# ahmetumutdurmus/zaremba

Hardware: NVIDIA H100
Metric: tokens/sec (and valid perplexity) Large-LSTM 1500h at 1/2/4/8 H100 vs ref CPU (higher is better)
Workload: dtype f16 operands, f32 accumulate/state

## Files before the change

### zaremba_b200/csrc/adam_tc.cu

```cuda
#include "update_tile.cuh"

namespace zrb {

__device__ __forceinline__ void adam_elem(float& p, float& g, float& m, float& v, float coef, const AdamScalars& k) {
    g = __fmul_rn(g, coef);
    m = __fadd_rn(__fmul_rn(k.beta1, m), __fmul_rn(k.omb1, g));
    v = __fadd_rn(__fmul_rn(k.beta2, v), __fmul_rn(k.omb2, __fmul_rn(g, g)));
    const float denom = __fadd_rn(__fdiv_rn(__fsqrt_rn(v), k.bc2s), k.eps);
    p = __fsub_rn(p, __fmul_rn(k.step_size, __fdiv_rn(m, denom)));
}

struct AdamRule : NoTileRule {
    float* m;
    float* v;
    AdamScalars k;
    const float* scalars;
    float coef;
    static constexpr bool kMayWriteG = true;
    static constexpr int kWhhMinBlocks = 3;
    template <int VEC> struct Tile { float m[kTileRows][VEC], v[kTileRows][VEC]; };
    __device__ __forceinline__ void init() { coef = scalars[1]; }
    template <int VEC>
    __device__ __forceinline__ void apply(int64_t, float (&)[VEC], float (&)[VEC]) const {}
    template <int VEC> __device__ __forceinline__ void load(int64_t off, int e, Tile<VEC>& t) const {
        load_vec<VEC>(m + off, t.m[e]);
        load_vec<VEC>(v + off, t.v[e]);
    }
    template <int VEC>
    __device__ __forceinline__ void finish(int e, float (&pv)[VEC], float (&gv)[VEC], Tile<VEC>& t) const {
#pragma unroll
        for (int x = 0; x < VEC; ++x) adam_elem(pv[x], gv[x], t.m[e][x], t.v[e][x], coef, k);
    }
    template <int VEC> __device__ __forceinline__ void store(int64_t off, int e, const Tile<VEC>& t) const {
        store_vec<VEC>(m + off, t.m[e]);
        store_vec<VEC>(v + off, t.v[e]);
    }
};

int update_pack_adam(float* p, float* g, float* m, float* v, const AdamScalars& k, int rows, int cols,
                     const float* scalars, const WeightImages& img, bool write_g, cudaStream_t s, bool pdl) {
    AdamRule rule;
    rule.m = m; rule.v = v; rule.k = k; rule.scalars = scalars; rule.coef = 0.f;
    return update_pack_rule(p, g, rows, cols, rule, (uintptr_t)m | (uintptr_t)v, img, write_g, s, pdl);
}

constexpr int kAdamListThreads = 256;
constexpr int kAdamListBlocks = 148 * 16;

struct AdamRuns {
    float* p[kMaxTensors];
    float* g[kMaxTensors];
    float* m[kMaxTensors];
    float* v[kMaxTensors];
    int64_t n[kMaxTensors];
};

template <bool WRITE_G>
__global__ void __launch_bounds__(kAdamListThreads) adam_list_kernel(AdamRuns d, AdamScalars k,
                                                                     const float* __restrict__ scalars) {
    float* __restrict__ p = d.p[blockIdx.y];
    float* __restrict__ g = d.g[blockIdx.y];
    float* __restrict__ m = d.m[blockIdx.y];
    float* __restrict__ v = d.v[blockIdx.y];
    const int64_t n = d.n[blockIdx.y];
    const float coef = scalars[1];
    const int64_t tid = (int64_t)blockIdx.x * blockDim.x + threadIdx.x, stride = (int64_t)gridDim.x * blockDim.x;
    int64_t j0 = 0;
    if (((((uintptr_t)p) | ((uintptr_t)g) | ((uintptr_t)m) | ((uintptr_t)v)) & 15) == 0) {
        const int64_t n4 = n >> 2;
        for (int64_t i = tid; i < n4; i += stride) {
            float pv[4], gv[4], mv[4], vv[4];
            load_vec<4>(g + 4 * i, gv);
            load_vec<4>(p + 4 * i, pv);
            load_vec<4>(m + 4 * i, mv);
            load_vec<4>(v + 4 * i, vv);
#pragma unroll
// ... 41 lines not shown
```

### zaremba_b200/csrc/average_tc.cu

```cuda
#include "update_tile.cuh"

namespace zrb {

__device__ __forceinline__ float avg_elem(float a, float p, float mu, int first) {
    return first ? p : __fadd_rn(a, __fmul_rn(__fsub_rn(p, a), mu));
}

struct AvgRule : SgdRule {
    float* a;
    float mu;
    int first;
    static constexpr int kWhhMinBlocks = 3;
    template <int VEC> struct Tile { float v[kTileRows][VEC]; };
    template <int VEC> __device__ __forceinline__ void load(int64_t off, int e, Tile<VEC>& t) const {
        load_vec<VEC>(a + off, t.v[e]);
    }
    template <int VEC>
    __device__ __forceinline__ void finish(int e, float (&pv)[VEC], float (&)[VEC], Tile<VEC>& t) const {
#pragma unroll
        for (int x = 0; x < VEC; ++x) t.v[e][x] = avg_elem(t.v[e][x], pv[x], mu, first);
    }
    template <int VEC> __device__ __forceinline__ void store(int64_t off, int e, const Tile<VEC>& t) const {
        store_vec<VEC>(a + off, t.v[e]);
    }
};

struct SwapRule : NoTileRule {
    static constexpr bool kMayWriteG = true;
    static constexpr int kWhhMinBlocks = 4;
    __device__ __forceinline__ void init() {}
    template <int VEC>
    __device__ __forceinline__ void apply(int64_t, float (&pv)[VEC], float (&gv)[VEC]) const {
#pragma unroll
        for (int x = 0; x < VEC; ++x) { const float t = pv[x]; pv[x] = gv[x]; gv[x] = t; }
    }
};

int update_pack_avg(float* p, float* g, float* a, float mu, bool first, int rows, int cols, float lr,
                    const float* scalars, const WeightImages& img, bool write_g, cudaStream_t s, bool pdl) {
    AvgRule rule;
    rule.lr = lr; rule.scalars = scalars; rule.coef = 0.f;
    rule.a = a; rule.mu = mu; rule.first = first ? 1 : 0;
    return update_pack_rule(p, g, rows, cols, rule, (uintptr_t)a, img, write_g, s, pdl);
}

int swap_pack(float* p, float* a, int rows, int cols, const WeightImages& img, cudaStream_t s) {
    return update_pack_rule(p, a, rows, cols, SwapRule{}, 0, img, true, s, false);
}

constexpr int kListThreads = 256;
constexpr int kListBlocks = 148 * 16;

struct AvgRuns {
    float* p[kMaxTensors];
    float* g[kMaxTensors];
    float* a[kMaxTensors];
    int64_t n[kMaxTensors];
};

static int avg_runs(const TensorList& tl, float* const* a, AvgRuns* d, int* bx) {
    int k = 0;
    int64_t longest = 0;
    for (int t = 0; t < tl.count; ++t) {
        if (tl.n[t] == 0) continue;
        d->p[k] = tl.p[t]; d->g[k] = tl.g[t]; d->a[k] = a[t]; d->n[k] = tl.n[t];
        longest = tl.n[t] > longest ? tl.n[t] : longest;
        ++k;
    }
    int64_t b = (longest / 4 + kListThreads - 1) / kListThreads;
    if (b < 1) b = 1;
    const int cap = kListBlocks / (k > 0 ? k : 1);
    *bx = (int)(b > cap ? cap : b);
    return k;
}

template <bool SGD, bool WRITE_G>
// ... 99 lines not shown
```

### zaremba_b200/csrc/engine_tc.cu

```cuda
#include "engine.h"
#include <stdlib.h>
#include <string.h>

#include "tc_kernels.h"

struct GridBarrier {
    unsigned int* word = nullptr;
    unsigned int base = 0;
    template <typename Launch>
    int claim(int T, int nCTA, cudaStream_t s, Launch&& launch) {
        const unsigned int arrivals = (unsigned int)T * (unsigned int)nCTA;
        if (base > 0xF0000000u - arrivals) {
            ZRB_CUDA(cudaMemsetAsync(word, 0, sizeof(unsigned int), s));
            base = 0;
        }
        ZRB_TRY(launch(word, base));
        base += arrivals;
        return ZRB_OK;
    }
};

struct zrb_tc_state {
    int Xp[ZRB_MAX_LAYERS + 1] = {}, G4p[ZRB_MAX_LAYERS] = {}, Vp = 0;
    int Fp = 0;
// ... 292 lines not shown
    }
    ms.m[ms.n++] = {1 + 4 * L, V, K ? c->width[0] : c->width[L], L, WeightMatrix::kFcW};
    return ms;
}
static WeightImages tc_images(zrb_ctx* c, const WeightMatrix& m, const zrb_tc_state::WhhImage& whh) {
    zrb_tc_state* t = c->tc;
    switch (m.kind) {
        case WeightMatrix::kWhh: return t->w_hh_images(m.item, whh);
        case WeightMatrix::kWih: return t->w_ih_images(m.item);
        case WeightMatrix::kFcW: return t->fc_w_images();
        case WeightMatrix::kPrior: return t->row_image(t->head_w_h + (size_t)t->Ua * t->Xp[m.item], t->Xp[m.item]);
        default: return t->row_image(t->head_w_h, t->Xp[m.item]);
    }
}
static TensorList tc_without_matrices(const zrb_ctx* c, const TensorList& tl) {
    TensorList rest = tl;
    for (const WeightMatrix& m : tc_matrices(c)) rest.n[m.i] = 0;
    return rest;
}
static bool tc_streams_aligned(const TensorList& tl, float* const* x1 = nullptr, float* const* x2 = nullptr) {
    uintptr_t all = 0;
    for (int i = 0; i < tl.count; ++i)
        all |= (uintptr_t)tl.p[i] | (uintptr_t)tl.g[i] | (x1 ? (uintptr_t)x1[i] : 0) | (x2 ? (uintptr_t)x2[i] : 0);
    return (all & 3) == 0;
}
static void tc_images_current(zrb_ctx* c, const zrb_params* p) {
    zrb_tc_state* t = c->tc;
    t->wg_ok = false;
    c->weights_version++;
    note_packed(c, p);
}

static int tc_update_matrix(zrb_ctx* c, const WeightMatrix& m, const TensorList& tl, float lr, const AvgStep* avg,
                            const AdamStep* adam, bool pdl, cudaStream_t s) {
    zrb_tc_state::WhhImage whh;
    if (c->p_wd > 0.f) whh.kind = zrb_tc_state::kWhhStale;
    const WeightImages img = tc_images(c, m, whh);
    float *p = tl.p[m.i], *g = tl.g[m.i];
    if (adam)
        return update_pack_adam(p, g, adam->m[m.i], adam->v[m.i], adam->k, m.rows, m.cols, c->scalars, img,
                                c->keep_clipped, s, pdl);
    if (!avg) return update_pack(p, g, m.rows, m.cols, lr, c->scalars, img, c->keep_clipped, s, pdl);
    return update_pack_avg(p, g, avg->a[m.i], avg->mu, avg->first, m.rows, m.cols, lr, c->scalars, img, c->keep_clipped,
                           s, pdl);
}

static int tc_issue_update(zrb_ctx* c, int item, bool pdl, cudaStream_t s) {
    zrb_tc_state* t = c->tc;
    if (!(t->upd_pending & (1u << item))) return ZRB_OK;
    t->upd_pending &= ~(1u << item);
    const AvgStep* avg = t->upd_avg_on ? &t->upd_avg : nullptr;
    const AdamStep* adam = t->upd_adam_on ? &t->upd_adam : nullptr;
    for (const WeightMatrix& m : tc_matrices(c))
        if (m.item == item) ZRB_TRY(tc_update_matrix(c, m, t->upd_tl, t->upd_lr, avg, adam, pdl, s));
    return ZRB_OK;
}

int tc_flush_updates(zrb_ctx* c, cudaStream_t s) {
    zrb_tc_state* t = c->tc;
    if (!t || !t->upd_pending) return ZRB_OK;
    ProfScope ps(c, ZRB_PROF_CLIP_SGD, s);
    for (int item = 1; item <= c->cfg.layers; ++item) ZRB_TRY(tc_issue_update(c, item, false, s));
    return ZRB_OK;
}

static int tc_mos_head(zrb_ctx* c, const zrb_params* p, int rows, float* logp, cudaStream_t s) {
    zrb_tc_state* t = c->tc;
    const int L = c->cfg.layers, V = c->cfg.vocab, K = c->experts, E = c->width[0], H = c->width[L];
    const int N = c->T * c->B, Xl = t->Xp[L], Ep = pad64(E);
    ProfScope ps(c, ZRB_PROF_PROJ_FWD, s);
    Gemm head;
    head.A = {t->x_h[L] + (size_t)(N - rows) * Xl, Xl}; head.B = {t->head_w_h, Xl};
    head.C = t->ua; head.ldc = t->HW; head.M = rows; head.N = t->Ua + K; head.K = H;
    ZRB_TRY(gemm_f16_tc(head, s));
    ZRB_TRY(mos_latent_fwd(t->ua, t->HW, mos_of(p)->latent_b, t->lat_h, Ep, rows, K, E, N - rows, mos_mask(c), s));
    Gemm logits;
    logits.A = {t->lat_h, Ep}; logits.B = {t->fc_w_h, t->Fp};
    logits.C = t->logits; logits.ldc = V; logits.M = rows * K; logits.N = V; logits.K = E; logits.bias = p->fc_b;
    ZRB_TRY(gemm_f16_tc(logits, s));
    ZRB_TRY(mos_lse(t->logits, rows * K, V, t->lse, s));
    if (logp) ZRB_TRY(mos_logp(t->logits, t->lse, t->ua, t->HW, t->Ua, rows, K, V, logp, V, s));
    return ZRB_OK;
}

int tc_forward(zrb_ctx* c, const zrb_params* p, const int64_t* x, const zrb_states* in, const zrb_states* out,
               float* scores, cudaStream_t s, bool last_only) {
    zrb_tc_state* t = c->tc;
    const int L = c->cfg.layers, V = c->cfg.vocab, T = c->T, B = c->B, N = T * B;
    const bool ride = t->upd_pending && t->in_train_step && t->fplan[0].ok && pdl_beside_rec(c);
    if (t->upd_pending && !ride) ZRB_TRY(tc_flush_updates(c, s));
    ZRB_TRY(tc_pack_weights(c, p, s));
    {
        FwdPrep fp = {};
        for (int l = 0; l < L; ++l) {
            fp.in_h[l] = in->h[l]; fp.in_c[l] = in->c[l]; fp.h0s[l] = c->h0s[l]; fp.c0s[l] = c->c0s[l];
// ... 12 lines not shown
        ZRB_TRY(embed_dropout_fwd(p->embed_w, x, nullptr, t->x_h[0], t->Xp[0], N, c->width[0], V, site_mask(c, 0), ed_mask(c), s,
                                  through ? t->upd_tl.g[tc_matrices(c).fc_w().i] : nullptr, t->upd_lr, c->scalars));
    }
    for (int l = 0; l < L; ++l) {
        const int In = c->width[l], H = c->width[l + 1], Xi = t->Xp[l], Hp = t->Xp[l + 1];
        const size_t bh = (size_t)B * H * sizeof(float);
        const RecPlan& fplan = t->fplan[l];
        float* G = c->gates[l];
        if (!whh_current(c, l)) {
            ProfScope ps(c, ZRB_PROF_PACK, s);
            ZRB_TRY(tc_pack_whh(c, p->w_hh[l], l, false, s));
        }
        {
            ProfScope ps(c, ZRB_PROF_GEMM_IN, s);
            Gemm xw;
            xw.A = {t->x_h[l], Xi}; xw.B = {t->w_ih_h[l], Xi};
            xw.C = G; xw.ldc = 4 * H; xw.M = N; xw.N = 4 * H; xw.K = In; xw.bias = p->b_ih[l]; xw.bias2 = p->b_hh[l];
            ZRB_TRY(gemm_f16_tc(xw, s));
        }
        MaskSrc m = site_mask(c, l + 1), rm = rec_mask(c, l);
        const ZoneoutSrc zo = zoneout_src(c, l);
        const bool reg_h = t->in_train_step && reg_on(c) && l == L - 1;
        ProfScope ps(c, ZRB_PROF_REC_FWD, s);
        if (fplan.ok) {
            ZRB_TRY(t->fwd_bar.claim(T, fplan.nCTA, s, [&](unsigned int* word, unsigned int base) {
                RecFwdArgs a = {};
                a.w_img = t->w_img_f[l]; a.h0_img = t->h0_img[l]; a.h_img = t->h_img; a.gates = G; a.c0 = c->c0s[l];
                a.cst = c->cst[l]; a.h_last = out->h[l]; a.c_last = out->c[l]; a.hprev_h = t->hprev_h[l];
                a.y_h = t->x_h[l + 1]; a.h_f32 = reg_h ? c->hraw[l] : nullptr; a.counter = word; a.base = base;
                a.T = T; a.B = B; a.H = H; a.Hp = Hp; a.m = m; a.rm = rm; a.trace = t->trace;
                a.zo = zo; a.h0 = c->h0s[l]; a.ctil = c->ctil[l];
                return lstm_rec_fwd(fplan, tc_watchdog(c), a, s);
            }));
            if (ride) ZRB_TRY(tc_issue_update(c, l + 1, true, s));
            continue;
        }
        for (int tt = 0; tt < T; ++tt) {
            const float* c_prev = tt ? c->cst[l] + (size_t)(tt - 1) * B * H : c->c0s[l];
            float* Gt = G + (size_t)tt * B * 4 * H;
            Gemm hw;
            hw.A = {t->hprev_h[l] + (size_t)tt * B * Hp, Hp}; hw.B = {t->w_hh_h[l], Hp};
            hw.C = Gt; hw.ldc = 4 * H; hw.M = B; hw.N = 4 * H; hw.K = H; hw.accumulate = true;
            ZRB_TRY(gemm_f16_tc(hw, s));
            const float* h_prev = tt ? c->hraw[l] + (size_t)(tt - 1) * B * H : c->h0s[l];
            ZRB_TRY(lstm_cell_fwd_tc(Gt, c_prev, c->cst[l] + (size_t)tt * B * H, c->hraw[l] + (size_t)tt * B * H,
                                     t->hprev_h[l] + (size_t)(tt + 1) * B * Hp, t->x_h[l + 1] + (size_t)tt * B * Hp, Hp, B,
                                     H, (int64_t)tt * B * H, (int64_t)N * H, m, rm, s, zo.on ? &zo : nullptr, h_prev,
                                     zo.on ? c->ctil[l] + (size_t)tt * B * H : nullptr));
        }
        ZRB_CUDA(cudaMemcpyAsync(out->h[l], c->hraw[l] + (size_t)(T - 1) * B * H, bh, cudaMemcpyDeviceToDevice, s));
        ZRB_CUDA(cudaMemcpyAsync(out->c[l], c->cst[l] + (size_t)(T - 1) * B * H, bh, cudaMemcpyDeviceToDevice, s));
    }
    if (scores && c->experts) return tc_mos_head(c, p, last_only ? B : N, t->head_loss_only ? nullptr : scores, s);
    if (scores) {
        ProfScope ps(c, ZRB_PROF_PROJ_FWD, s);
        const int rows = last_only ? B : N;
        const int Xl = t->Xp[L];
        Gemm proj;
        proj.A = {t->x_h[L] + (size_t)(N - rows) * Xl, Xl}; proj.B = {t->fc_w_h, Xl};
        proj.C = scores; proj.ldc = V; proj.M = rows; proj.N = V; proj.K = c->width[L]; proj.bias = p->fc_b;
        ZRB_TRY(gemm_f16_tc(proj, s));
    }
    return ZRB_OK;
}

const __half* tc_last_layer_image(const zrb_ctx* c) { return c->tc->x_h[c->cfg.layers]; }

// ... 418 lines not shown
    TensorList rest = tc_without_matrices(c, tl);
    if (rows_only && !adam) rest.n[0] = 0;
    TensorList dense = gemm_norm ? rest : tl;
    if (rows_only) dense.n[0] = 0;
    if (c->tied && gemm_norm) {
        ZRB_TRY(grad_norm(dense, max_norm, c->partials, c->scalars, norm_out, s, true, t->wg_slots));
    } else if (rows_only) {
        ZRB_TRY(embed_first_table(c->emb_prev_ids, c->emb_first, c->emb_prev_n, V, s));
        ZRB_TRY(embed_rows_sumsq(tl.g[0], c->emb_prev_ids, c->emb_first, c->emb_prev_n, E, V,
                                 c->partials + norm_partials_base(), kNormExtra, s));
        ZRB_TRY(grad_norm(dense, max_norm, c->partials, c->scalars, norm_out, s, true, gemm_norm ? t->wg_slots : 0));
        if (!adam)
            ZRB_TRY(embed_rows_update(tl.p[0], tl.g[0], c->emb_prev_ids, c->emb_first, c->emb_prev_n, E, V, lr,
                                      c->scalars, c->keep_clipped, s));
        if (avg) {
            TensorList e{};
            e.p[0] = tl.p[0]; e.n[0] = tl.n[0]; e.count = 1;
            ZRB_TRY(avg_apply(e, avg->a, avg->mu, avg->first, s));
        }
    } else {
        ZRB_TRY(grad_norm(tl, max_norm, c->partials, c->scalars, norm_out, s));
    }
    const bool lazy = c->lazy_update && t->persistent() && pdl_beside_rec(c);
    if (lazy) {
        t->upd_tl = tl;
        t->upd_lr = lr;
        t->upd_avg_on = avg != nullptr;
        if (avg) t->upd_avg = *avg;
        t->upd_adam_on = adam != nullptr;
        if (adam) t->upd_adam = *adam;
    }
    for (const WeightMatrix& m : tc_matrices(c)) {
        if (lazy && m.item >= 1 && !(adam && c->tied && m.item == L)) t->upd_pending |= 1u << m.item;
        else ZRB_TRY(tc_update_matrix(c, m, tl, lr, avg, adam, false, s));
    }
    if (adam) ZRB_TRY(adam_apply(rest, *adam, c->scalars, c->keep_clipped, s));
    else if (avg) ZRB_TRY(sgd_avg_apply(rest, avg->a, lr, c->scalars, c->keep_clipped, avg->mu, avg->first, s));
    else ZRB_TRY(sgd_apply(rest, lr, c->scalars, c->keep_clipped, s));
    tc_images_current(c, p);
    return ZRB_OK;
}

int tc_dyneval_update(zrb_ctx* c, const zrb_params* p, const TensorList& tl, float* const* tg, float* const* r,
                      const DynArgs& a, cudaStream_t s) {
    ZRB_TRY(tc_flush_updates(c, s));
    ProfScope ps(c, ZRB_PROF_CLIP_SGD, s);
    if (!tc_streams_aligned(tl, tg, r)) {
        ZRB_TRY(dyneval_apply(tl, tg, r, a, s));
        c->weights_version++;
        return ZRB_OK;
    }
    for (const WeightMatrix& m : tc_matrices(c))
        ZRB_TRY(update_pack_dyn(tl.p[m.i], tl.g[m.i], tg[m.i], r ? r[m.i] : nullptr, m.rows, m.cols, a,
                                tc_images(c, m, {}), s));
    ZRB_TRY(dyneval_apply(tc_without_matrices(c, tl), tg, r, a, s));
    tc_images_current(c, p);
    return ZRB_OK;
}

int tc_swap_average(zrb_ctx* c, const zrb_params* p, const TensorList& tl, float* const* a, cudaStream_t s) {
    ZRB_TRY(tc_flush_updates(c, s));
    ProfScope ps(c, ZRB_PROF_PACK, s);
    if (!tc_streams_aligned(tl, a)) {
        ZRB_TRY(swap_apply(tl, a, s));
        c->weights_version++;
        return ZRB_OK;
    }
// ... 8 lines not shown
```

### zaremba_b200/csrc/lstm_rec_bwd.cu

```cuda
#include <stdlib.h>

#include "lstm_rec_bwd.cuh"

namespace zrb {

__global__ void pack_whh_bwd_kernel(const float* __restrict__ W, __half* __restrict__ img, int H, int UC, int G, int KcS,
                                    int S, int nCluster, MaskSrc m) {
    __shared__ __half tile[8][8 * 128];
    const int warp_in_block = threadIdx.x >> 5, lane = threadIdx.x & 31;
    const int CS = 4 * S;
    const long long total = (long long)nCluster * CS * KcS;
    for (long long w = (long long)blockIdx.x * 8 + warp_in_block; w < total; w += (long long)gridDim.x * 8) {
        const int kcl = (int)(w % KcS);
        const int r = (int)((w / KcS) % CS);
        const int cl = (int)(w / ((long long)KcS * CS));
        const int gate = r / S, khalf = r % S;
        __half* t = tile[warp_in_block];
        const int rows8 = G * 8;
        if (m.active) {
            for (int idx = lane * 4; idx < 8 * rows8; idx += 128) {
                const int e = idx / rows8, u0 = idx % rows8;
                const int k = (khalf * KcS + kcl) * 8 + e, j0 = cl * UC + u0;
                const size_t row = (size_t)gate * H + k;
                float mul[4] = {0.f, 0.f, 0.f, 0.f};
                if (k < H && u0 < UC && j0 < H) mask_mul4_at(m, row * H + j0, mul);
#pragma unroll
                for (int q = 0; q < 4; ++q) {
                    const int u = u0 + q, j = j0 + q;
                    t[u * 8 + e] = __float2half_rn((k < H && u < UC && j < H) ? W[row * H + j] * mul[q] : 0.f);
                }
            }
        } else {
            for (int idx = lane; idx < 8 * rows8; idx += 32) {
                int e = idx / rows8, u = idx % rows8;
                int k = (khalf * KcS + kcl) * 8 + e, j = cl * UC + u;
                float v = (k < H && u < UC && j < H) ? W[((size_t)gate * H + k) * H + j] : 0.f;
                t[u * 8 + e] = __float2half_rn(v);
            }
        }
        __syncwarp();
        __half* dst = img + (((size_t)cl * CS + r) * KcS + kcl) * ((size_t)G * 64);
        for (int idx = lane; idx < rows8 * 8; idx += 32) dst[idx] = t[idx];
        __syncwarp();
    }
}

int rec_bwd_plan(int H, int B, RecPlan* plan) {
    int nsm = tc_num_sms();
    plan->GB = (B + 7) / 8;
    plan->ok = 0;
    plan->KS = 1;
    if (plan->GB * 8 > 32) return ZRB_OK;
    if (H >= 256) {
        const int Kp = (H + 31) / 32 * 32, Kc = Kp / 8, KcS = Kc / 2, GBi = (plan->GB + 1) / 2 * 2;
        for (int pass = 0; pass < 2; ++pass)
            for (int U = 16; U >= 1; --U) {
                const int UC = 8 * U;
                if (UC > 128) continue;
                const int ncl = (H + UC - 1) / UC;
                if (ncl * 8 > nsm) break;
                if (U * B > (pass == 0 ? 1 : kRecMaxCell) * kRecEpiThreads) continue;
                const int G = UC / 8;
                const size_t smem = rec_smem_bytes(KcS, G, GBi);
                if (smem <= 227 * 1024 && 8 * U * (GBi * 8 + 4) <= 2 * 64 * (GBi * 8 + 1)) {
                    if (rec_max_clusters((const void*)lstm_rec_bwd_kernel<2, false>, 8, (int)smem, 8 * 64) < ncl) continue;
                    plan->KS = 2; plan->U = U; plan->G = G; plan->nCTA = ncl * 8; plan->smem = (int)smem;
                    plan->Kc = Kc; plan->KcS = KcS; plan->GBi = GBi;
                    return rec_plan_finish(plan, (const void*)lstm_rec_bwd_kernel<2, false>, 8);
                }
            }
    }
    int Kp = (H + 15) / 16 * 16;
    plan->Kc = Kp / 8;
    plan->KcS = plan->Kc;
    plan->GBi = plan->GB;
    int max_clusters = (nsm - 16) / 4;
    for (int U = 16; U >= 1; --U) {
        int UC = 4 * U;
        if (UC % 8) continue;
        int ncl = (H + UC - 1) / UC;
        if (ncl > max_clusters) break;
        int G = UC / 8;
        size_t smem = rec_smem_bytes(plan->Kc, G, plan->GB);
        if (smem <= 227 * 1024 && U * B <= kRecMaxCell * kRecEpiThreads) {
            plan->U = U; plan->G = G; plan->nCTA = ncl * 4; plan->smem = (int)smem;
            return rec_plan_finish(plan, (const void*)lstm_rec_bwd_kernel<1, false>, 4);
        }
    }
    return ZRB_OK;
}

int pack_whh_bwd(const float* W, __half* img, int H, const RecPlan& p, cudaStream_t s, MaskSrc m) {
    const int CS = 4 * p.KS;
    pack_whh_bwd_kernel<<<tc_num_sms() * 4, 256, 0, s>>>(W, img, H, CS * p.U, p.G, p.KcS, p.KS, p.nCTA / CS, m);
// ... 23 lines not shown
```

### zaremba_b200/csrc/lstm_rec_fwd.cu

```cuda
#include <stdlib.h>

#include "lstm_rec_fwd.cuh"

namespace zrb {

__global__ void pack_whh_fwd_kernel(const float* __restrict__ W, __half* __restrict__ img, int H, int UC, int G, int KcS,
                                    int KS, int nCTA, MaskSrc m) {
    const size_t per_cta = (size_t)KcS * G * 64;
    const size_t total = per_cta * nCTA;
    if (m.active) {
        for (size_t idx = ((size_t)blockIdx.x * blockDim.x + threadIdx.x) * 4; idx < total;
             idx += (size_t)gridDim.x * blockDim.x * 4) {
            int cta = (int)(idx / per_cta);
            size_t r0 = idx % per_cta;
            int e0 = (int)(r0 & 7), r = (int)((r0 >> 3) & 7);
            int g = (int)((r0 >> 6) % G), kcl = (int)((r0 >> 6) / G);
            int i = g * 8 + r, uc = i >> 2, q = i & 3;
            int cluster = cta / KS, rank = cta % KS;
            int j = cluster * UC + uc, k0 = (rank * KcS + kcl) * 8 + e0;
            const bool row_ok = uc < UC && j < H;
            const size_t row = (size_t)q * H + j;
            float mul[4] = {0.f, 0.f, 0.f, 0.f};
            if (row_ok && k0 < H) mask_mul4_at(m, row * H + k0, mul);
#pragma unroll
            for (int t = 0; t < 4; ++t)
                img[idx + t] = __float2half_rn(row_ok && k0 + t < H ? W[row * H + k0 + t] * mul[t] : 0.f);
        }
        return;
    }
    for (size_t idx = (size_t)blockIdx.x * blockDim.x + threadIdx.x; idx < total;
         idx += (size_t)gridDim.x * blockDim.x) {
        int cta = (int)(idx / per_cta);
        size_t r0 = idx % per_cta;
        int e = (int)(r0 & 7), r = (int)((r0 >> 3) & 7);
        int g = (int)((r0 >> 6) % G), kcl = (int)((r0 >> 6) / G);
        int i = g * 8 + r, uc = i >> 2, q = i & 3;
        int cluster = cta / KS, rank = cta % KS;
        int j = cluster * UC + uc, k = (rank * KcS + kcl) * 8 + e;
        float v = 0.f;
        if (uc < UC && j < H && k < H) v = W[((size_t)q * H + j) * H + k];
        img[idx] = __float2half_rn(v);
    }
}

size_t rec_smem_bytes(int Kc, int G, int GB) {
    return (size_t)Kc * G * 128 + (size_t)Kc * GB * 128 + 2 * 64 * (GB * 8 + 1) * 4 + 128  + 128 ;
}

int rec_max_clusters(const void* kernel, int cluster, int smem, int nCTA) {
    cudaLaunchConfig_t cfg = {};
    cfg.gridDim = dim3(nCTA);
    cfg.blockDim = dim3(kRecThreads);
    cfg.dynamicSmemBytes = (size_t)smem;
    cudaLaunchAttribute at[1];
    at[0].id = cudaLaunchAttributeClusterDimension;
    at[0].val.clusterDim.x = cluster; at[0].val.clusterDim.y = 1; at[0].val.clusterDim.z = 1;
    cfg.attrs = at; cfg.numAttrs = 1;
    int n = 0;
    if (cudaFuncSetAttribute(kernel, cudaFuncAttributeMaxDynamicSharedMemorySize, 227 * 1024) != cudaSuccess ||
        cudaOccupancyMaxActiveClusters(&n, kernel, &cfg) != cudaSuccess) {
        (void)cudaGetLastError();
        return 0;
    }
    return n;
}

int rec_plan_finish(RecPlan* plan, const void* kernel, int cluster) {
    plan->kernel = kernel;
    plan->cluster = cluster;
    plan->max_clusters = rec_max_clusters(kernel, cluster, plan->smem, plan->nCTA);
    plan->ok = 1;
    return ZRB_OK;
}

static bool rec_no_coop() {
    static const bool v = getenv("ZRB_NO_COOP") != nullptr || getenv("CUDA_INJECTION64_PATH") != nullptr ||
                          getenv("NV_COMPUTE_PROFILER_PERFWORKS_DIR") != nullptr || getenv("NVTX_INJECTION64_PATH") != nullptr;
    return v;
}

int rec_launch(const RecPlan& p, void** args, bool trace, cudaStream_t s, const char* name) {
    if (p.cluster == 1) {
        ZRB_CUDA(cudaLaunchCooperativeKernel(p.kernel, dim3(p.nCTA), dim3(kRecThreads), args, (size_t)p.smem, s));
        count_launch();
        return ZRB_OK;
    }
    int dev = 0;
    cudaGetDevice(&dev);
    cudaLaunchConfig_t cfg = {};
    cfg.gridDim = dim3(p.nCTA);
    cfg.blockDim = dim3(kRecThreads);
    cfg.dynamicSmemBytes = (size_t)p.smem;
    cfg.stream = s;
    cudaLaunchAttribute attrs[2];
    attrs[0].id = cudaLaunchAttributeClusterDimension;
    attrs[0].val.clusterDim.x = p.cluster; attrs[0].val.clusterDim.y = 1; attrs[0].val.clusterDim.z = 1;
    cfg.attrs = attrs;
    const bool programmatic = rec_launch_programmatic(dev) && !trace;
    const bool plain = programmatic || rec_no_coop();
    cudaError_t e = cudaSuccess;
    if (!plain) {
        attrs[1].id = cudaLaunchAttributeCooperative;
        attrs[1].val.cooperative = 1;
// ... 7 lines not shown
        if (e != cudaSuccess) (void)cudaGetLastError();
    }
    if (plain || e != cudaSuccess) {
        if (p.max_clusters * p.cluster < p.nCTA) {
            set_error("%s: %d clusters of %d needed, the device can hold %d at once", name, p.nCTA / p.cluster, p.cluster,
                      p.max_clusters);
            return ZRB_E_CUDA;
        }
        cfg.numAttrs = 1;
        if (programmatic) {
            attrs[1].id = cudaLaunchAttributeProgrammaticStreamSerialization;
            attrs[1].val.programmaticStreamSerializationAllowed = 1;
            cfg.numAttrs = 2;
        }
        e = cudaLaunchKernelExC(&cfg, p.kernel, args);
    }
    if (e != cudaSuccess) {
        set_error("%s launch failed: %s", name, cudaGetErrorString(e));
        return ZRB_E_CUDA;
    }
    count_launch();
    return ZRB_OK;
}

int rec_fwd_plan(int H, int B, RecPlan* plan) {
    const void* const kernel[2] = {(const void*)lstm_rec_fwd_kernel<false, false>,
                                   (const void*)lstm_rec_fwd_kernel<true, false>};
    int nsm = tc_num_sms();
    plan->GB = (B + 7) / 8;
    plan->ok = 0;
    plan->KS = 1;
    if (plan->GB * 8 > 32) return ZRB_OK;
    if (H >= 256) {
        const int Kp = (H + 31) / 32 * 32, Kc = Kp / 8, KcS = Kc / 2, GBi = (plan->GB + 1) / 2 * 2;
        for (int pass = 0; pass < 2; ++pass)
            for (int U = 16; U >= 1; --U) {
                const int npair = (H + 2 * U - 1) / (2 * U);
                if (2 * npair > nsm) break;
                if (U * B > (pass == 0 ? 1 : kRecMaxCell) * kRecEpiThreads) continue;
                const int G = U;
                const size_t smem = rec_smem_bytes(KcS, G, GBi);
                if (smem <= 227 * 1024 && 2 * 4 * U * (GBi * 8 + 4) <= 2 * 64 * (GBi * 8 + 1)) {
                    plan->KS = 2; plan->U = U; plan->G = G; plan->nCTA = 2 * npair; plan->smem = (int)smem;
                    plan->Kc = Kc; plan->KcS = KcS; plan->GBi = GBi;
                    return rec_plan_finish(plan, kernel[1], 2);
                }
            }
    }
    int Kp = (H + 15) / 16 * 16;
    plan->Kc = Kp / 8;
    plan->KcS = plan->Kc;
    plan->GBi = plan->GB;
    for (int U = 16; U >= 1; --U) {
        int n = (H + U - 1) / U;
        if (n > nsm) break;
        int G = (4 * U + 7) / 8;
        size_t smem = rec_smem_bytes(plan->Kc, G, plan->GB);
        if (smem <= 227 * 1024 && U * B <= kRecMaxCell * kRecEpiThreads) {
            plan->U = U; plan->G = G; plan->nCTA = n; plan->smem = (int)smem;
            return rec_plan_finish(plan, kernel[0], 1);
        }
    }
    return ZRB_OK;
}

int pack_whh_fwd(const float* W, __half* img, int H, const RecPlan& p, cudaStream_t s, MaskSrc m) {
    pack_whh_fwd_kernel<<<tc_num_sms() * 4, 256, 0, s>>>(W, img, H, p.KS * p.U, p.G, p.KcS, p.KS, p.nCTA, m);
    ZRB_KERNEL_CHECK();
    return ZRB_OK;
}

int lstm_rec_fwd(const RecPlan& p, const RecWatchdog& wd, RecFwdArgs a, cudaStream_t s) {
// ... 16 lines not shown
```

### zaremba_b200/csrc/optim_tc.cu

```cuda
#include "update_tile.cuh"

namespace zrb {

template <bool RMS>
struct DynRule : NoTileRule {
    const float* tg;
    const float* r;
    DynArgs a;
    float rbar;
    static constexpr bool kMayWriteG = false;
    static constexpr int kWhhMinBlocks = 4;
    __device__ __forceinline__ void init() { rbar = RMS ? *a.rbar : 0.f; }
    template <int VEC>
    __device__ __forceinline__ void apply(int64_t off, float (&pv)[VEC], float (&gv)[VEC]) const {
        float tv[VEC], rv[VEC];
        load_vec<VEC>(tg + off, tv);
        if constexpr (RMS) load_vec<VEC>(r + off, rv);
#pragma unroll
        for (int x = 0; x < VEC; ++x)
            pv[x] = dyneval_elem<RMS>(pv[x], gv[x], tv[x], RMS ? rv[x] : 0.f, a.lr, a.lam, a.eps, rbar);
    }
};

int update_pack(float* p, float* g, int rows, int cols, float lr, const float* scalars, const WeightImages& img,
                bool write_g, cudaStream_t s, bool pdl) {
    SgdRule rule;
    rule.lr = lr; rule.scalars = scalars; rule.coef = 0.f;
    return update_pack_rule(p, g, rows, cols, rule, 0, img, write_g, s, pdl);
}

int update_pack_dyn(float* p, float* g, const float* tg, const float* r, int rows, int cols, const DynArgs& a,
                    const WeightImages& img, cudaStream_t s) {
    const uintptr_t align = ((uintptr_t)tg) | ((uintptr_t)r);
    if (a.rbar) {
        DynRule<true> rule{{}, tg, r, a, 0.f};
        return update_pack_rule(p, g, rows, cols, rule, align, img, false, s, false);
    }
    DynRule<false> rule{{}, tg, nullptr, a, 0.f};
    return update_pack_rule(p, g, rows, cols, rule, align, img, false, s, false);
}

}
```

### zaremba_b200/csrc/rec_common.cuh

```cuda
#pragma once
#include <string.h>
#include "tc_common.cuh"
#include "tc_kernels.h"

namespace zrb {
using namespace tc;

constexpr int kRecEpiWarps = 8;
constexpr int kRecEpiThreads = kRecEpiWarps * 32;
constexpr int kRecMmaWarp = 8;
constexpr int kRecMmaWarps = 4;
constexpr int kRecMmaThreads = kRecMmaWarps * 32;
constexpr int kRecLoadWarp = kRecMmaWarp + kRecMmaWarps;
constexpr int kRecThreads = (kRecLoadWarp + 1) * 32;
constexpr int kRecPieces = 4;
constexpr int kRecMaxCell = 2;
static inline RecWatch rec_watch_args(const RecWatchdog& wd) {
    static const long long spin = [] { const char* e = getenv("ZRB_SPIN_CYCLES"); long long v = e ? atoll(e) : 0; return v > 0 ? v : 6000000000ll; }();
    RecWatch w;
    w.flag = wd.flag; w.host = wd.host; w.spin_cycles = spin;
    return w;
}
static inline unsigned int rec_fault_base(const char* which) {
    static const char* fault = getenv("ZRB_FAULT_BARRIER_BASE");
    return (fault && !strcmp(fault, which)) ? 1u : 0u;
}
enum { kWaitWeights = 1, kWaitOperand = 2, kWaitAcc = 3, kWaitRecv = 4, kWaitGrid = 5 };

__device__ __forceinline__ unsigned int ld_relaxed_gpu(const unsigned int* p) {
    unsigned int v;
    asm volatile("ld.relaxed.gpu.global.u32 %0, [%1];" : "=r"(v) : "l"(p) : "memory");
    return v;
}
static __device__ __noinline__ void rec_give_up(unsigned int* flag, unsigned int* host, int kind, int step) {
    const unsigned int code = (unsigned int)kind | ((unsigned int)(blockIdx.x & 0xFFF) << 8) | ((unsigned int)(step & 0xFFF) << 20);
    if (atomicCAS(flag, 0u, code) == 0u) {
        asm volatile("st.relaxed.sys.global.u32 [%0], %1;" ::"l"(host), "r"(code) : "memory");
        __threadfence_system();
    }
}
__device__ __forceinline__ bool rec_spin_expired(const RecWatch& w, long long& t0) {
    if (ld_relaxed_gpu(w.flag) != 0u) return true;
    const long long now = clock64();
    if (t0 == 0) { t0 = now; return false; }
    return now - t0 > w.spin_cycles;
}
__device__ __forceinline__ bool rec_spin_check(const RecWatch& w, long long& t0, int kind, int step) {
    if (!rec_spin_expired(w, t0)) return false;
    rec_give_up(w.flag, w.host, kind, step);
// ... 147 lines not shown
```

### zaremba_b200/csrc/tc_kernels.h

```cpp
#pragma once
#include "kernels.h"
#include "tc_host.h"

namespace zrb {

constexpr float kGradScale = 1024.f;

int convert_pad_f16(const float* src, int64_t ld_src, __half* dst, int64_t ld_dst, int rows, int cols, float scale,
                    cudaStream_t s, MaskSrc m = MaskSrc{});
int colsum_h_scratch_floats(int M);
int colsum_h(const __half* A, int64_t ld, float* out, float* out2, int N, int M, float inv_scale, float* scratch,
             cudaStream_t s);

int mos_latent_fwd(float* ua, int64_t ldu, const float* b, __half* lat_h, int64_t ld_l, int rows, int K, int E,
                   int64_t row0, MaskSrc m, cudaStream_t s);
int mos_latent_bwd(const float* dlat, const float* ua, int64_t ldu, __half* dua_h, int64_t ld_d, int N, int K, int E,
                   MaskSrc m, cudaStream_t s);
int mos_lse(const float* Z, int rows, int V, float* lse, cudaStream_t s);
int mos_nll_grad(const float* Z, const float* lse, const float* ua, int64_t ldu, int Ua, const int64_t* y, int N, int K,
                 int V, int B, float* row_loss, float* loss, __half* ds_h, int64_t ld_s, __half* dua_h, int64_t ld_d,
                 cudaStream_t s);
int mos_nll_eval(const float* Z, const float* lse, const float* ua, int64_t ldu, int Ua, const int64_t* y, int N, int K,
                 int V, int B, float* row_loss, float* loss, float* tgt_prob, cudaStream_t s);
int mos_logp(const float* Z, const float* lse, const float* ua, int64_t ldu, int Ua, int rows, int K, int V, float* out,
// ... 1 lines not shown
int mos_vjp(const float* Z, const float* lse, const float* ua, int64_t ldu, int Ua, int N, int K, int V, const float* G,
            float* P, float* s_buf, __half* ds_h, int64_t ld_s, __half* dua_h, int64_t ld_d, cudaStream_t s);

struct ZoneoutSrc;
int lstm_cell_fwd_tc(float* pre, const float* c_prev, float* c_out, float* h_raw, __half* h_raw_h, __half* y_h,
                     int64_t ld_h, int B, int H, int64_t elem_off, int64_t n_total, MaskSrc m, MaskSrc rm, cudaStream_t s,
                     const ZoneoutSrc* zo = nullptr, const float* h_prev = nullptr, float* c_til = nullptr);
int lstm_cell_bwd_tc(const float* dy_post, const float* dh_rec, float* dc, const float* gates, const float* c_t,
                     const float* c_prev, float* dG, __half* dG_h, int64_t ld_g, int B, int H, int64_t elem_off,
                     int64_t n_total, MaskSrc m, MaskSrc rm, cudaStream_t s, const float* r = nullptr,
                     const ZoneoutSrc* zo = nullptr, float* hcarry = nullptr);

struct ZoneoutSrc {
    const uint8_t* flags;
    float ec, ec1, eh, eh1;
    int on;
};
int zoneout_flags(MaskSrc c, MaskSrc h, int64_t n, uint8_t* flags, cudaStream_t s);

struct RecPlan {
    int ok;
    int U;
    int G;
    int GB;
    int Kc;
    int nCTA;
    int smem;
    int KS;
    int KcS;
    int GBi;
    const void* kernel;
    int cluster;
    int max_clusters;
};
size_t rec_smem_bytes(int Kc, int G, int GB);
int rec_max_clusters(const void* kernel, int cluster, int smem, int nCTA);
int rec_plan_finish(RecPlan* plan, const void* kernel, int cluster);
int rec_launch(const RecPlan& p, void** args, bool trace, cudaStream_t s, const char* name);
const void* rec_fwd_zoneout_kernel(bool split);
const void* rec_bwd_zoneout_kernel(int S);
struct RecWatchdog {
    unsigned int* flag = nullptr;
    unsigned int* host = nullptr;
};
struct RecWatch {
    unsigned int* flag;
    unsigned int* host;
    long long spin_cycles;
};
int rec_fwd_plan(int H, int B, RecPlan* plan);
int pack_whh_fwd(const float* W, __half* img, int H, const RecPlan& p, cudaStream_t s, MaskSrc m = MaskSrc{});
struct RecFwdArgs {
    const __half* w_img;
    const __half* h0_img;
    __half* h_img;
    float* gates;
    const float* c0;
    float* cst;
    float* h_last;
    float* c_last;
    __half* hprev_h;
    __half* y_h;
    float* h_f32;
    unsigned int* counter;
    unsigned int base;
    int T, B, H, Hp, U, G, GB, Kc, nCTA;
    int KcS, GBi;
    MaskSrc m;
    MaskSrc rm;
    RecWatch w;
    long long* trace;
    ZoneoutSrc zo;
    const float* h0;
    float* ctil;
};
int lstm_rec_fwd(const RecPlan& p, const RecWatchdog& wd, RecFwdArgs a, cudaStream_t s);
struct FwdPrep {
    const float* in_h[ZRB_MAX_LAYERS];
    const float* in_c[ZRB_MAX_LAYERS];
    float* h0s[ZRB_MAX_LAYERS];
    float* c0s[ZRB_MAX_LAYERS];
    __half* hprev_h[ZRB_MAX_LAYERS];
    __half* h0_img[ZRB_MAX_LAYERS];
    MaskSrc rm[ZRB_MAX_LAYERS];
    const int64_t* x;
    int64_t* x_saved;
    int H[ZRB_MAX_LAYERS], Hp[ZRB_MAX_LAYERS];
    int GB[ZRB_MAX_LAYERS], Kc[ZRB_MAX_LAYERS];
    int L, B, N;
};
int fwd_prep(const FwdPrep& a, cudaStream_t s);
struct WeightImages {
    __half* row = nullptr;
    int64_t ld = 0;
    __half* fwd = nullptr;
    const RecPlan* fplan = nullptr;
    __half* bwd = nullptr;
    const RecPlan* bplan = nullptr;
};
int update_pack(float* p, float* g, int rows, int cols, float lr, const float* scalars, const WeightImages& img,
                bool write_g, cudaStream_t s,
                bool pdl = false);
int update_pack_dyn(float* p, float* g, const float* tg, const float* r, int rows, int cols, const DynArgs& a,
                    const WeightImages& img, cudaStream_t s);
int update_pack_avg(float* p, float* g, float* a, float mu, bool first, int rows, int cols, float lr,
                    const float* scalars, const WeightImages& img, bool write_g, cudaStream_t s, bool pdl = false);
int update_pack_adam(float* p, float* g, float* m, float* v, const AdamScalars& k, int rows, int cols,
                     const float* scalars, const WeightImages& img, bool write_g, cudaStream_t s, bool pdl = false);
int swap_pack(float* p, float* a, int rows, int cols, const WeightImages& img, cudaStream_t s);
int rec_bwd_plan(int H, int B, RecPlan* plan);
int pack_whh_bwd(const float* W, __half* img, int H, const RecPlan& p, cudaStream_t s, MaskSrc m = MaskSrc{});
struct RecBwdArgs {
    const __half* w_img;
    __half* g_img;
    const float* dy;
    const float* r;
    const float* gates;
    const float* cst;
    const float* c0;
    __half* dG_h;
    float* db1;
    float* db2;
    float* db_scratch;
    unsigned int* counter;
    unsigned int base;
    int T, B, H, G4p, U, G, GB, Kc, nCTA;
    int KcS, GBi;
    MaskSrc m;
    MaskSrc rm;
    RecWatch w;
    long long* trace;
    ZoneoutSrc zo;
    const float* ctil;
};
int lstm_rec_bwd(const RecPlan& p, const RecWatchdog& wd, RecBwdArgs a, cudaStream_t s);

}
```

### zaremba_b200/csrc/update_tile.cuh

```cuda
#pragma once
#include "tc_kernels.h"

namespace zrb {

struct PackSpec {
    __half* row_img;
    int64_t ld;
    __half* fwd_img;
    int fU, fG, fKc, fKS;
    __half* bwd_img;
    int bUC, bG, bKc, bS;
    int write_g;
    int pdl;
};

__device__ __forceinline__ void pdl_prologue(const PackSpec& sp) {
    if (sp.pdl && threadIdx.x == 0) asm volatile("griddepcontrol.launch_dependents;" ::: "memory");
}
__device__ __forceinline__ void pdl_epilogue(const PackSpec& sp) {
    if (sp.pdl && blockIdx.x == 0 && threadIdx.x == 0) asm volatile("griddepcontrol.wait;" ::: "memory");
}

template <int VEC> struct VecT;
template <> struct VecT<4> { using type = float4; };
// ... 193 lines not shown
        }
        const unsigned rank = q * sp.bS + jb / (unsigned)sp.bKc, kcl = jb - (jb / sp.bKc) * sp.bKc;
        __half* base = sp.bwd_img + (int64_t)kcl * sp.bG * 64;
        auto put = [&](int unit, const uint4& val) {
            if (unit < H) {
                const unsigned cl = (unsigned)unit / (unsigned)sp.bUC, u = unit - cl * sp.bUC;
                st_v4(base + (int64_t)((cl * 4 * sp.bS + rank) * sp.bKc) * sp.bG * 64 + (u >> 3) * 64 + (u & 7) * 8, val);
            }
        };
        if constexpr (VEC == 1) {
            put(c, v[0]);
        } else {
            const bool lower = ((lane >> 2) & 1) == 0;
            const int a = lower ? c : c - VEC;
            uint4 recv[VEC / 2];
#pragma unroll
            for (int m = 0; m < VEC / 2; ++m) {
                const uint4 s = lower ? v[2 * m + 1] : v[2 * m];
                recv[m] = make_uint4(__shfl_xor_sync(0xffffffffu, s.x, 4), __shfl_xor_sync(0xffffffffu, s.y, 4),
                                     __shfl_xor_sync(0xffffffffu, s.z, 4), __shfl_xor_sync(0xffffffffu, s.w, 4));
            }
#pragma unroll
            for (int i = 0; i < VEC; ++i) {
                if (lower) put(a + 2 * i, i < VEC / 2 ? v[2 * i] : recv[i - VEC / 2]);
                else put(a + 2 * i + 1, i < VEC / 2 ? recv[i] : v[2 * (i - VEC / 2) + 1]);
            }
        }
    }
    pdl_epilogue(sp);
}

template <int VEC, class Rule>
static int update_pack_launch(float* p, float* g, int rows, int cols, const Rule& rule, const PackSpec& sp, bool whh,
                              cudaStream_t s) {
    const int cv = cols / VEC;
    int threads = kUpdThreads, col_tiles;
    if (whh) {
        col_tiles = (cv + 8 * (threads / 32) - 1) / (8 * (threads / 32));
    } else {
        threads = min(kUpdThreads, (cv + 31) / 32 * 32);
        col_tiles = (cv + threads - 1) / threads;
    }
    const dim3 grid((unsigned)(((rows / (whh ? 4 : 1)) + kTileRows - 1) / kTileRows * col_tiles));
    if (sp.pdl) {
        cudaLaunchConfig_t cfg = {};
        cfg.gridDim = grid; cfg.blockDim = dim3(threads); cfg.dynamicSmemBytes = 12 * 1024; cfg.stream = s;
        cudaLaunchAttribute at[1];
        at[0].id = cudaLaunchAttributeProgrammaticStreamSerialization;
        at[0].val.programmaticStreamSerializationAllowed = 1;
        cfg.attrs = at; cfg.numAttrs = 1;
        if (whh) ZRB_CUDA(cudaLaunchKernelEx(&cfg, update_pack_whh_kernel<VEC, Rule>, p, g, cols, col_tiles, rule, sp));
        else ZRB_CUDA(cudaLaunchKernelEx(&cfg, update_pack_kernel<VEC, Rule>, p, g, rows, cols, col_tiles, rule, sp));
        count_launch();
        return ZRB_OK;
    }
    if (whh) update_pack_whh_kernel<VEC, Rule><<<grid, threads, 0, s>>>(p, g, cols, col_tiles, rule, sp);
    else update_pack_kernel<VEC, Rule><<<grid, threads, 0, s>>>(p, g, rows, cols, col_tiles, rule, sp);
    ZRB_KERNEL_CHECK();
    return ZRB_OK;
}

template <class Rule>
static int update_pack_rule(float* p, float* g, int rows, int cols, const Rule& rule, uintptr_t align,
                            const WeightImages& img, bool write_g, cudaStream_t s, bool pdl) {
    const RecPlan *fp = img.fplan, *bp = img.bplan;
    PackSpec sp;
    sp.write_g = write_g ? 1 : 0;
    sp.pdl = pdl ? 1 : 0;
    sp.row_img = img.row; sp.ld = img.ld;
    sp.fwd_img = img.fwd; sp.fKS = fp ? fp->KS : 1; sp.fU = fp ? fp->KS * fp->U : 1; sp.fG = fp ? fp->G : 1;
    sp.fKc = fp ? fp->KcS : 1;
    sp.bwd_img = img.bwd; sp.bS = bp ? bp->KS : 1; sp.bUC = bp ? 4 * bp->KS * bp->U : 4; sp.bG = bp ? bp->G : 1;
    sp.bKc = bp ? bp->KcS : 1;
    const bool whh = (img.fwd || img.bwd) && rows == 4 * cols;
    const uintptr_t all = ((uintptr_t)p) | ((uintptr_t)g) | align;
    const bool al16 = (all & 15) == 0, al8 = (all & 7) == 0;
    if (cols % 4 == 0 && al16) return update_pack_launch<4>(p, g, rows, cols, rule, sp, whh, s);
    if (cols % 2 == 0 && al8) return update_pack_launch<2>(p, g, rows, cols, rule, sp, whh, s);
    return update_pack_launch<1>(p, g, rows, cols, rule, sp, whh, s);
}

}
```

Measured before the change: 403,500.

## Size overlapped update smem to fit beside recurrent kernel and reserve SMs for it

The PDL-launched weight update kernel that rides alongside the forward recurrent kernel now requests dynamic shared memory computed from the recurrent plan (per-SM smem minus the recurrent kernel's smem plus one byte), instead of a fixed 12KB. This is meant to stop it from co-residing on SMs occupied by the persistent recurrent CTAs. The split-K plan selection also changes: first-pass choices now require the CTA count to leave about an eighth of SMs free, so the update kernel has somewhere to run. GB rounding to even becomes a minimum of 2. The risk is fewer SMs for the recurrence, and an update kernel that may wait for free SMs.

```diff
diff --git a/zaremba_b200/csrc/adam_tc.cu b/zaremba_b200/csrc/adam_tc.cu
--- a/zaremba_b200/csrc/adam_tc.cu
+++ b/zaremba_b200/csrc/adam_tc.cu
@@ -38,10 +38,10 @@
 };
 
 int update_pack_adam(float* p, float* g, float* m, float* v, const AdamScalars& k, int rows, int cols,
-                     const float* scalars, const WeightImages& img, bool write_g, cudaStream_t s, bool pdl) {
+                     const float* scalars, const WeightImages& img, bool write_g, cudaStream_t s, int pdl_smem) {
     AdamRule rule;
     rule.m = m; rule.v = v; rule.k = k; rule.scalars = scalars; rule.coef = 0.f;
-    return update_pack_rule(p, g, rows, cols, rule, (uintptr_t)m | (uintptr_t)v, img, write_g, s, pdl);
+    return update_pack_rule(p, g, rows, cols, rule, (uintptr_t)m | (uintptr_t)v, img, write_g, s, pdl_smem);
 }
 
 constexpr int kAdamListThreads = 256;
diff --git a/zaremba_b200/csrc/average_tc.cu b/zaremba_b200/csrc/average_tc.cu
--- a/zaremba_b200/csrc/average_tc.cu
+++ b/zaremba_b200/csrc/average_tc.cu
@@ -37,11 +37,11 @@
 };
 
 int update_pack_avg(float* p, float* g, float* a, float mu, bool first, int rows, int cols, float lr,
-                    const float* scalars, const WeightImages& img, bool write_g, cudaStream_t s, bool pdl) {
+                    const float* scalars, const WeightImages& img, bool write_g, cudaStream_t s, int pdl_smem) {
     AvgRule rule;
     rule.lr = lr; rule.scalars = scalars; rule.coef = 0.f;
     rule.a = a; rule.mu = mu; rule.first = first ? 1 : 0;
-    return update_pack_rule(p, g, rows, cols, rule, (uintptr_t)a, img, write_g, s, pdl);
+    return update_pack_rule(p, g, rows, cols, rule, (uintptr_t)a, img, write_g, s, pdl_smem);
 }
 
 int swap_pack(float* p, float* a, int rows, int cols, const WeightImages& img, cudaStream_t s) {
diff --git a/zaremba_b200/csrc/engine_tc.cu b/zaremba_b200/csrc/engine_tc.cu
--- a/zaremba_b200/csrc/engine_tc.cu
+++ b/zaremba_b200/csrc/engine_tc.cu
@@ -348,27 +348,27 @@
 }
 
 static int tc_update_matrix(zrb_ctx* c, const WeightMatrix& m, const TensorList& tl, float lr, const AvgStep* avg,
-                            const AdamStep* adam, bool pdl, cudaStream_t s) {
+                            const AdamStep* adam, int pdl_smem, cudaStream_t s) {
     zrb_tc_state::WhhImage whh;
     if (c->p_wd > 0.f) whh.kind = zrb_tc_state::kWhhStale;
     const WeightImages img = tc_images(c, m, whh);
     float *p = tl.p[m.i], *g = tl.g[m.i];
     if (adam)
         return update_pack_adam(p, g, adam->m[m.i], adam->v[m.i], adam->k, m.rows, m.cols, c->scalars, img,
-                                c->keep_clipped, s, pdl);
-    if (!avg) return update_pack(p, g, m.rows, m.cols, lr, c->scalars, img, c->keep_clipped, s, pdl);
+                                c->keep_clipped, s, pdl_smem);
+    if (!avg) return update_pack(p, g, m.rows, m.cols, lr, c->scalars, img, c->keep_clipped, s, pdl_smem);
     return update_pack_avg(p, g, avg->a[m.i], avg->mu, avg->first, m.rows, m.cols, lr, c->scalars, img, c->keep_clipped,
-                           s, pdl);
-}
-
-static int tc_issue_update(zrb_ctx* c, int item, bool pdl, cudaStream_t s) {
+                           s, pdl_smem);
+}
+
+static int tc_issue_update(zrb_ctx* c, int item, int pdl_smem, cudaStream_t s) {
     zrb_tc_state* t = c->tc;
     if (!(t->upd_pending & (1u << item))) return ZRB_OK;
     t->upd_pending &= ~(1u << item);
     const AvgStep* avg = t->upd_avg_on ? &t->upd_avg : nullptr;
     const AdamStep* adam = t->upd_adam_on ? &t->upd_adam : nullptr;
     for (const WeightMatrix& m : tc_matrices(c))
-        if (m.item == item) ZRB_TRY(tc_update_matrix(c, m, t->upd_tl, t->upd_lr, avg, adam, pdl, s));
+        if (m.item == item) ZRB_TRY(tc_update_matrix(c, m, t->upd_tl, t->upd_lr, avg, adam, pdl_smem, s));
     return ZRB_OK;
 }
 
@@ -376,7 +376,7 @@
     zrb_tc_state* t = c->tc;
     if (!t || !t->upd_pending) return ZRB_OK;
     ProfScope ps(c, ZRB_PROF_CLIP_SGD, s);
-    for (int item = 1; item <= c->cfg.layers; ++item) ZRB_TRY(tc_issue_update(c, item, false, s));
+    for (int item = 1; item <= c->cfg.layers; ++item) ZRB_TRY(tc_issue_update(c, item, 0, s));
     return ZRB_OK;
 }
 
@@ -455,7 +455,7 @@
                 a.zo = zo; a.h0 = c->h0s[l]; a.ctil = c->ctil[l];
                 return lstm_rec_fwd(fplan, tc_watchdog(c), a, s);
             }));
-            if (ride) ZRB_TRY(tc_issue_update(c, l + 1, true, s));
+            if (ride) ZRB_TRY(tc_issue_update(c, l + 1, fplan.beside_smem, s));
             continue;
         }
         for (int tt = 0; tt < T; ++tt) {
@@ -940,7 +940,7 @@
     }
     for (const WeightMatrix& m : tc_matrices(c)) {
         if (lazy && m.item >= 1 && !(adam && c->tied && m.item == L)) t->upd_pending |= 1u << m.item;
-        else ZRB_TRY(tc_update_matrix(c, m, tl, lr, avg, adam, false, s));
+        else ZRB_TRY(tc_update_matrix(c, m, tl, lr, avg, adam, 0, s));
     }
     if (adam) ZRB_TRY(adam_apply(rest, *adam, c->scalars, c->keep_clipped, s));
     else if (avg) ZRB_TRY(sgd_avg_apply(rest, avg->a, lr, c->scalars, c->keep_clipped, avg->mu, avg->first, s));
diff --git a/zaremba_b200/csrc/lstm_rec_bwd.cu b/zaremba_b200/csrc/lstm_rec_bwd.cu
--- a/zaremba_b200/csrc/lstm_rec_bwd.cu
+++ b/zaremba_b200/csrc/lstm_rec_bwd.cu
@@ -52,14 +52,15 @@
     plan->KS = 1;
     if (plan->GB * 8 > 32) return ZRB_OK;
     if (H >= 256) {
-        const int Kp = (H + 31) / 32 * 32, Kc = Kp / 8, KcS = Kc / 2, GBi = (plan->GB + 1) / 2 * 2;
+        const int Kp = (H + 31) / 32 * 32, Kc = Kp / 8, KcS = Kc / 2, GBi = rec_split_groups(plan->GB);
         for (int pass = 0; pass < 2; ++pass)
             for (int U = 16; U >= 1; --U) {
                 const int UC = 8 * U;
                 if (UC > 128) continue;
                 const int ncl = (H + UC - 1) / UC;
                 if (ncl * 8 > nsm) break;
-                if (U * B > (pass == 0 ? 1 : kRecMaxCell) * kRecEpiThreads) continue;
+                if (U * B > kRecMaxCell * kRecEpiThreads || (pass == 0 && !rec_split_first_choice(U, B, 8 * ncl, nsm)))
+                    continue;
                 const int G = UC / 8;
                 const size_t smem = rec_smem_bytes(KcS, G, GBi);
                 if (smem <= 227 * 1024 && 8 * U * (GBi * 8 + 4) <= 2 * 64 * (GBi * 8 + 1)) {
diff --git a/zaremba_b200/csrc/lstm_rec_fwd.cu b/zaremba_b200/csrc/lstm_rec_fwd.cu
--- a/zaremba_b200/csrc/lstm_rec_fwd.cu
+++ b/zaremba_b200/csrc/lstm_rec_fwd.cu
@@ -47,6 +47,8 @@
     return (size_t)Kc * G * 128 + (size_t)Kc * GB * 128 + 2 * 64 * (GB * 8 + 1) * 4 + 128  + 128 ;
 }
 
+int rec_split_groups(int GB) { return GB < 2 ? 2 : GB; }
+
 int rec_max_clusters(const void* kernel, int cluster, int smem, int nCTA) {
     cudaLaunchConfig_t cfg = {};
     cfg.gridDim = dim3(nCTA);
@@ -69,6 +71,11 @@
     plan->kernel = kernel;
     plan->cluster = cluster;
     plan->max_clusters = rec_max_clusters(kernel, cluster, plan->smem, plan->nCTA);
+    int dev = 0, per_sm = 0, reserved = 0;
+    ZRB_CUDA(cudaGetDevice(&dev));
+    ZRB_CUDA(cudaDeviceGetAttribute(&per_sm, cudaDevAttrMaxSharedMemoryPerMultiprocessor, dev));
+    ZRB_CUDA(cudaDeviceGetAttribute(&reserved, cudaDevAttrReservedSharedMemoryPerBlock, dev));
+    plan->beside_smem = per_sm - 2 * reserved - plan->smem + 1;
     plan->ok = 1;
     return ZRB_OK;
 }
@@ -142,12 +149,13 @@
     plan->KS = 1;
     if (plan->GB * 8 > 32) return ZRB_OK;
     if (H >= 256) {
-        const int Kp = (H + 31) / 32 * 32, Kc = Kp / 8, KcS = Kc / 2, GBi = (plan->GB + 1) / 2 * 2;
+        const int Kp = (H + 31) / 32 * 32, Kc = Kp / 8, KcS = Kc / 2, GBi = rec_split_groups(plan->GB);
         for (int pass = 0; pass < 2; ++pass)
             for (int U = 16; U >= 1; --U) {
                 const int npair = (H + 2 * U - 1) / (2 * U);
                 if (2 * npair > nsm) break;
-                if (U * B > (pass == 0 ? 1 : kRecMaxCell) * kRecEpiThreads) continue;
+                if (U * B > kRecMaxCell * kRecEpiThreads || (pass == 0 && !rec_split_first_choice(U, B, 2 * npair, nsm)))
+                    continue;
                 const int G = U;
                 const size_t smem = rec_smem_bytes(KcS, G, GBi);
                 if (smem <= 227 * 1024 && 2 * 4 * U * (GBi * 8 + 4) <= 2 * 64 * (GBi * 8 + 1)) {
diff --git a/zaremba_b200/csrc/optim_tc.cu b/zaremba_b200/csrc/optim_tc.cu
--- a/zaremba_b200/csrc/optim_tc.cu
+++ b/zaremba_b200/csrc/optim_tc.cu
@@ -23,10 +23,10 @@
 };
 
 int update_pack(float* p, float* g, int rows, int cols, float lr, const float* scalars, const WeightImages& img,
-                bool write_g, cudaStream_t s, bool pdl) {
+                bool write_g, cudaStream_t s, int pdl_smem) {
     SgdRule rule;
     rule.lr = lr; rule.scalars = scalars; rule.coef = 0.f;
-    return update_pack_rule(p, g, rows, cols, rule, 0, img, write_g, s, pdl);
+    return update_pack_rule(p, g, rows, cols, rule, 0, img, write_g, s, pdl_smem);
 }
 
 int update_pack_dyn(float* p, float* g, const float* tg, const float* r, int rows, int cols, const DynArgs& a,
diff --git a/zaremba_b200/csrc/rec_common.cuh b/zaremba_b200/csrc/rec_common.cuh
--- a/zaremba_b200/csrc/rec_common.cuh
+++ b/zaremba_b200/csrc/rec_common.cuh
@@ -15,6 +15,9 @@
 constexpr int kRecThreads = (kRecLoadWarp + 1) * 32;
 constexpr int kRecPieces = 4;
 constexpr int kRecMaxCell = 2;
+inline bool rec_split_first_choice(int U, int B, int nCTA, int nsm) {
+    return U * B <= kRecEpiThreads && nCTA <= nsm - nsm / 8;
+}
 static inline RecWatch rec_watch_args(const RecWatchdog& wd) {
     static const long long spin = [] { const char* e = getenv("ZRB_SPIN_CYCLES"); long long v = e ? atoll(e) : 0; return v > 0 ? v : 6000000000ll; }();
     RecWatch w;
diff --git a/zaremba_b200/csrc/tc_kernels.h b/zaremba_b200/csrc/tc_kernels.h
--- a/zaremba_b200/csrc/tc_kernels.h
+++ b/zaremba_b200/csrc/tc_kernels.h
@@ -57,8 +57,10 @@
     const void* kernel;
     int cluster;
     int max_clusters;
+    int beside_smem;
 };
 size_t rec_smem_bytes(int Kc, int G, int GB);
+int rec_split_groups(int GB);
 int rec_max_clusters(const void* kernel, int cluster, int smem, int nCTA);
 int rec_plan_finish(RecPlan* plan, const void* kernel, int cluster);
 int rec_launch(const RecPlan& p, void** args, bool trace, cudaStream_t s, const char* name);
@@ -125,13 +127,13 @@
 };
 int update_pack(float* p, float* g, int rows, int cols, float lr, const float* scalars, const WeightImages& img,
                 bool write_g, cudaStream_t s,
-                bool pdl = false);
+                int pdl_smem = 0);
 int update_pack_dyn(float* p, float* g, const float* tg, const float* r, int rows, int cols, const DynArgs& a,
                     const WeightImages& img, cudaStream_t s);
 int update_pack_avg(float* p, float* g, float* a, float mu, bool first, int rows, int cols, float lr,
-                    const float* scalars, const WeightImages& img, bool write_g, cudaStream_t s, bool pdl = false);
+                    const float* scalars, const WeightImages& img, bool write_g, cudaStream_t s, int pdl_smem = 0);
 int update_pack_adam(float* p, float* g, float* m, float* v, const AdamScalars& k, int rows, int cols,
-                     const float* scalars, const WeightImages& img, bool write_g, cudaStream_t s, bool pdl = false);
+                     const float* scalars, const WeightImages& img, bool write_g, cudaStream_t s, int pdl_smem = 0);
 int swap_pack(float* p, float* a, int rows, int cols, const WeightImages& img, cudaStream_t s);
 int rec_bwd_plan(int H, int B, RecPlan* plan);
 int pack_whh_bwd(const float* W, __half* img, int H, const RecPlan& p, cudaStream_t s, MaskSrc m = MaskSrc{});
diff --git a/zaremba_b200/csrc/update_tile.cuh b/zaremba_b200/csrc/update_tile.cuh
--- a/zaremba_b200/csrc/update_tile.cuh
+++ b/zaremba_b200/csrc/update_tile.cuh
@@ -249,7 +249,7 @@
 
 template <int VEC, class Rule>
 static int update_pack_launch(float* p, float* g, int rows, int cols, const Rule& rule, const PackSpec& sp, bool whh,
-                              cudaStream_t s) {
+                              int pdl_smem, cudaStream_t s) {
     const int cv = cols / VEC;
     int threads = kUpdThreads, col_tiles;
     if (whh) {
@@ -259,15 +259,22 @@
         col_tiles = (cv + threads - 1) / threads;
     }
     const dim3 grid((unsigned)(((rows / (whh ? 4 : 1)) + kTileRows - 1) / kTileRows * col_tiles));
-    if (sp.pdl) {
+    if (pdl_smem > 0) {
         cudaLaunchConfig_t cfg = {};
-        cfg.gridDim = grid; cfg.blockDim = dim3(threads); cfg.dynamicSmemBytes = 12 * 1024; cfg.stream = s;
+        cfg.gridDim = grid; cfg.blockDim = dim3(threads); cfg.dynamicSmemBytes = (size_t)pdl_smem; cfg.stream = s;
         cudaLaunchAttribute at[1];
         at[0].id = cudaLaunchAttributeProgrammaticStreamSerialization;
         at[0].val.programmaticStreamSerializationAllowed = 1;
         cfg.attrs = at; cfg.numAttrs = 1;
-        if (whh) ZRB_CUDA(cudaLaunchKernelEx(&cfg, update_pack_whh_kernel<VEC, Rule>, p, g, cols, col_tiles, rule, sp));
-        else ZRB_CUDA(cudaLaunchKernelEx(&cfg, update_pack_kernel<VEC, Rule>, p, g, rows, cols, col_tiles, rule, sp));
+        if (whh) {
+            ZRB_CUDA(cudaFuncSetAttribute(update_pack_whh_kernel<VEC, Rule>, cudaFuncAttributeMaxDynamicSharedMemorySize,
+                                          pdl_smem));
+            ZRB_CUDA(cudaLaunchKernelEx(&cfg, update_pack_whh_kernel<VEC, Rule>, p, g, cols, col_tiles, rule, sp));
+        } else {
+            ZRB_CUDA(cudaFuncSetAttribute(update_pack_kernel<VEC, Rule>, cudaFuncAttributeMaxDynamicSharedMemorySize,
+                                          pdl_smem));
+            ZRB_CUDA(cudaLaunchKernelEx(&cfg, update_pack_kernel<VEC, Rule>, p, g, rows, cols, col_tiles, rule, sp));
+        }
         count_launch();
         return ZRB_OK;
     }
@@ -279,11 +286,11 @@
 
 template <class Rule>
 static int update_pack_rule(float* p, float* g, int rows, int cols, const Rule& rule, uintptr_t align,
-                            const WeightImages& img, bool write_g, cudaStream_t s, bool pdl) {
+                            const WeightImages& img, bool write_g, cudaStream_t s, int pdl_smem) {
     const RecPlan *fp = img.fplan, *bp = img.bplan;
     PackSpec sp;
     sp.write_g = write_g ? 1 : 0;
-    sp.pdl = pdl ? 1 : 0;
+    sp.pdl = pdl_smem > 0 ? 1 : 0;
     sp.row_img = img.row; sp.ld = img.ld;
     sp.fwd_img = img.fwd; sp.fKS = fp ? fp->KS : 1; sp.fU = fp ? fp->KS * fp->U : 1; sp.fG = fp ? fp->G : 1;
     sp.fKc = fp ? fp->KcS : 1;
@@ -292,9 +299,9 @@
     const bool whh = (img.fwd || img.bwd) && rows == 4 * cols;
     const uintptr_t all = ((uintptr_t)p) | ((uintptr_t)g) | align;
     const bool al16 = (all & 15) == 0, al8 = (all & 7) == 0;
-    if (cols % 4 == 0 && al16) return update_pack_launch<4>(p, g, rows, cols, rule, sp, whh, s);
-    if (cols % 2 == 0 && al8) return update_pack_launch<2>(p, g, rows, cols, rule, sp, whh, s);
-    return update_pack_launch<1>(p, g, rows, cols, rule, sp, whh, s);
-}
-
-}
+    if (cols % 4 == 0 && al16) return update_pack_launch<4>(p, g, rows, cols, rule, sp, whh, pdl_smem, s);
+    if (cols % 2 == 0 && al8) return update_pack_launch<2>(p, g, rows, cols, rule, sp, whh, pdl_smem, s);
+    return update_pack_launch<1>(p, g, rows, cols, rule, sp, whh, pdl_smem, s);
+}
+
+}
```

After: 439,400, median of 6. 8.9% higher.
